# eth-cscs/conflux

Measured on AMD Instinct MI355X. Metric: fp64_lu_tflops, higher is better.
Workload: dtype f64; 1 GPU; conflux LU N=16384 v=512 grid 1x1x1 (BASELINE cfg for 1 GPU); N=16384, v=512, grid=1x1x1

## Files before the change

### conflux_amd/__init__.py

```python
import ctypes
import os

_HERE = os.path.dirname(os.path.abspath(__file__))
_LIB_PATH = os.path.join(_HERE, "libconflux_lu.so")

UID_BYTES = 128


class ConfluxLuError(RuntimeError):
    pass


def _load():
    if not os.path.exists(_LIB_PATH):
        raise ConfluxLuError(
            f"HIP engine not built: {_LIB_PATH} missing. "
            "Run `make -C conflux_amd` (or __graft_entry__.build()). "
            "The product has no CPU fallback.")
    lib = ctypes.CDLL(_LIB_PATH)
    lib.conflux_lu_create.argtypes = [ctypes.c_int] * 7 + [
        ctypes.c_char_p, ctypes.POINTER(ctypes.c_void_p)]
    lib.conflux_lu_make_uid.argtypes = [ctypes.c_char_p]
    lib.conflux_lu_init_matrix.argtypes = [ctypes.c_void_p, ctypes.c_uint64]
    lib.conflux_lu_init_matrix_spd.argtypes = [ctypes.c_void_p, ctypes.c_uint64]
# ... 7 lines not shown
    lib.conflux_lu_factor.argtypes = [ctypes.c_void_p,
                                      ctypes.POINTER(ctypes.c_double)]
    lib.conflux_lu_get_factors.argtypes = [ctypes.c_void_p, ctypes.c_void_p,
                                           ctypes.c_void_p]
    lib.conflux_lu_get_factors_sim.argtypes = [ctypes.c_void_p, ctypes.c_int,
                                               ctypes.c_void_p, ctypes.c_void_p]
    lib.conflux_lu_dims.argtypes = [ctypes.c_void_p] + [
        ctypes.POINTER(ctypes.c_int)] * 6
    lib.conflux_lu_kernel_stats.argtypes = [
        ctypes.c_void_p, ctypes.c_int, ctypes.POINTER(ctypes.c_double),
        ctypes.POINTER(ctypes.c_long), ctypes.POINTER(ctypes.c_double)]
    lib.conflux_lu_validate.argtypes = [ctypes.c_void_p,
                                        ctypes.POINTER(ctypes.c_double)]
    lib.conflux_chol_validate.argtypes = [ctypes.c_void_p,
                                          ctypes.POINTER(ctypes.c_double)]
    lib.conflux_lu_destroy.argtypes = [ctypes.c_void_p]
    lib.conflux_lu_build_info.restype = ctypes.c_char_p
    lib.conflux_lu_debug_dgemm.argtypes = [
        ctypes.c_int, ctypes.c_longlong, ctypes.c_int, ctypes.c_void_p,
        ctypes.c_void_p, ctypes.c_void_p]
    lib.conflux_lu_debug_getrf.argtypes = [ctypes.c_int, ctypes.c_int,
                                           ctypes.c_void_p, ctypes.c_void_p]
    lib.conflux_lu_debug_set_panel_glue.argtypes = [ctypes.c_int]
    lib.conflux_lu_debug_set_trsm_stripe.argtypes = [ctypes.c_int]
    lib.conflux_lu_debug_trsm_stripe_width.argtypes = []
    lib.conflux_lu_debug_trsm_ld.argtypes = [
        ctypes.c_int, ctypes.c_int, ctypes.c_int, ctypes.c_longlong,
        ctypes.c_longlong, ctypes.c_longlong, ctypes.c_void_p,
        ctypes.c_void_p]
    lib.conflux_lu_debug_dgemm_bench.argtypes = [
        ctypes.c_int, ctypes.c_longlong, ctypes.c_int, ctypes.c_int,
        ctypes.POINTER(ctypes.c_double)]
    lib.conflux_lu_debug_trsm.argtypes = [
        ctypes.c_int, ctypes.c_int, ctypes.c_longlong, ctypes.c_int,
        ctypes.c_void_p, ctypes.c_void_p]
    lib.conflux_lu_solve.argtypes = [
        ctypes.c_void_p, ctypes.c_void_p, ctypes.c_int,
        ctypes.POINTER(ctypes.c_double)]
    lib.conflux_chol_solve.argtypes = lib.conflux_lu_solve.argtypes
    lib.conflux_lu_debug_trsm_left.argtypes = [
        ctypes.c_int, ctypes.c_int, ctypes.c_int, ctypes.c_longlong,
        ctypes.c_longlong, ctypes.c_void_p, ctypes.c_void_p]
    lib.conflux_lu_debug_update_skinny.argtypes = [
        ctypes.c_int, ctypes.c_int, ctypes.c_int, ctypes.c_longlong,
        ctypes.c_void_p, ctypes.c_void_p, ctypes.c_void_p]
    lib.conflux_lu_solve_refined.argtypes = [
# ... 267 lines not shown
```

### conflux_amd/csrc/engine.cpp

```cpp
#include <hip/hip_runtime.h>
#include <rccl/rccl.h>

#include <algorithm>
#include <chrono>
#include <cmath>
#include <cstdio>
#include <cstdlib>
#include <cstring>
#include <functional>
#include <numeric>
#include <string>
#include <set>
#include <vector>

#include "../../include/conflux_lu.h"
#include "kernels.hpp"
#include "norm1est.hpp"

#define HIPCHK(x)                                                       \
    do {                                                                \
        hipError_t e_ = (x);                                            \
        if (e_ != hipSuccess) {                                         \
            std::fprintf(stderr, "[conflux_lu] HIP error %s at %s:%d\n", \
                         hipGetErrorString(e_), __FILE__, __LINE__);    \
// ... 188 lines not shown
        if (!std::isfinite(x)) {
            ++bad;
            continue;
        }
        const double a = std::fabs(x);
        if (a == 0) ++zeros;
        if (a > mx) mx = a;
        if (a < mn) mn = a;
    }
    std::fprintf(stderr,
                 "[nanscan] k=%d %-12s bad=%ld/%lld zeros=%ld min=%.3e "
                 "max=%.3e\n",
                 k, tag, bad, (long long)ns, zeros, mn, mx);
}

int g_panel_glue = -1;
int panel_glue_mode() {
    if (g_panel_glue < 0) {
        const char *e = getenv("CONFLUX_PANEL_GLUE");
        g_panel_glue = e ? (atoi(e) != 0) : 1;
    }
    return g_panel_glue;
}

int factor_panel(Ctx &c, RankState &r, int n, std::vector<int> &ipiv_out) {
    const int v = c.v;
    const int NB = conflux_panel_nb();
    const int nsteps = std::min(v, n);
    ipiv_out.assign(v, 0);
    size_t slot;
    if (ev_begin(c, 1, 0, &slot)) return CONFLUX_LU_EHIP;
    auto leaf = [&](int jb, bool perm = true) -> int {
        const int nb = std::min(NB, nsteps - jb);
        const int m = n - jb;
        if (launch_panel_factor(r.panel + i64(jb) * v + jb, v, m, nb, r.sync,
                                r.d_ipiv + jb, c.epoch, r.d_swap,
                                r.d_swap + 64, c.stream)) {
            c.err = "panel grid not resident";
            return CONFLUX_LU_EINTERNAL;
        }
        c.epoch += nb;
        if (perm && v > nb)
            launch_rowperm_skip(r.panel, v, r.d_swap, r.d_swap + 64, jb,
                                2 * nb, jb, nb, v - nb, r.rowtmp, c.stream);
        return 0;
    };
// ... 58 lines not shown
                static int glue_cap = -1;
                if (glue_cap < 0) {
                    const char *gc = getenv("CONFLUX_GLUE_CAP");
                    glue_cap = gc ? atoi(gc) : 0;
                }
                launch_dgemm_f64(r.panel + i64(jb + nb) * v + jb, v,
                                 r.panel + i64(jb) * v + jb + nb, v,
                                 r.panel + i64(jb + nb) * v + jb + nb, v,
                                 m - nb, v - jb - nb, nb, c.stream,
                                 glue_cap);
            }
        }
    }
    if (ev_end(c, slot)) return CONFLUX_LU_EHIP;
    std::vector<int> raw(v);
    unsigned int perr = 0;
    char *d_err = (char *)r.sync + conflux_panel_err_offset();
    HIPCHK(hipMemcpyAsync(raw.data(), r.d_ipiv, nsteps * 4,
                          hipMemcpyDeviceToHost, c.stream));
    HIPCHK(hipMemcpyAsync(&perr, d_err, 4, hipMemcpyDeviceToHost, c.stream));
    HIPCHK(hipStreamSynchronize(c.stream));
    if (perr) {
        HIPCHK(hipMemsetAsync(d_err, 0, 4, c.stream));
        c.err = "panel hand-off timed out: column code " +
                std::to_string(perr) + " (1 + sub-panel column)";
        return CONFLUX_LU_EINTERNAL;
    }
    for (int jb = 0; jb < nsteps; jb += NB) {
        const int nb = std::min(NB, nsteps - jb);
        for (int s = 0; s < nb; ++s) ipiv_out[jb + s] = jb + raw[jb + s];
    }
    return 0;
}

void ipiv_to_perm(const std::vector<int> &ipiv, int n, int v,
                  std::vector<int> &perm) {
    perm.resize(std::max(2 * v, n));
    std::iota(perm.begin(), perm.end(), 0);
    for (int i = 0; i < std::min(v, n); ++i) std::swap(perm[i], perm[ipiv[i]]);
}

int g_trsm_stripe = -1;
int trsm_stripe_mode() {
    if (g_trsm_stripe < 0) {
        const char *e = getenv("CONFLUX_TRSM_STRIPE");
        g_trsm_stripe = e ? (atoi(e) != 0) : 1;
    }
    return g_trsm_stripe;
}
// ... 327 lines not shown
    int rc = timed_region(c, elapsed_ms, [&]() -> int {
        StepPlan sp;
        int rc = phase01(c, 0, sp);
        if (rc) return rc;
        for (int k = 0; k < c.Nt; ++k) {
            rc = run_step(c, k, sp);
            if (rc) return rc;
        }
        return 0;
    });
    if (rc) return rc;
    static int spin_stats = -1;
    if (spin_stats < 0) {
        const char *e = getenv("CONFLUX_SPIN_STATS");
        spin_stats = e ? atoi(e) : 0;
    }
    if (spin_stats) {
        for (auto &r : c.rs) {
            unsigned long long sp2 = 0;
            conflux_panel_spin_read(r.sync, &sp2, c.stream);
            std::fprintf(stderr, "[spinstats] rank %d spins=%llu\n",
                         r.grank, sp2);
        }
    }
    if (gap_stats_on())
        std::fprintf(stderr,
                     "[gapstats] steps=%ld entry->trsm=%.3f ms  gri/igri=%.3f "
                     "ms  entry->ev_pc=%.3f ms (%ld steps)\n",
                     g_gap.steps, g_gap.to_trsm, g_gap.gri, g_gap.to_evpc,
                     g_gap.evpc_steps);
    return 0;
}

int phase01(Ctx &c, int k, StepPlan &sp) {
    const int v = c.v, Px = c.Px, Py = c.Py, Pz = c.Pz;
    const int64_t Nl = c.Nl;
    const int loff = (k / Py) * v;
    const int kcol = k % Py, krow = k % Px;
    const int n_rounds = Px > 1 ? (int)std::ceil(std::log2((double)Px)) : 0;

    for (auto &r : c.rs) {
        if (r.pj != kcol) continue;
        launch_copy2d(r.A11 + i64(r.fnp) * Nl + loff, Nl,
                      r.A10 + i64(r.fnp) * v, v, r.nact, v, c.stream);
    }
    {
// ... 2114 lines not shown
    hipEvent_t a, b;
    HIPCHK(hipEventCreate(&a));
    HIPCHK(hipEventCreate(&b));
    HIPCHK(hipEventRecord(a, s));
    for (int i = 0; i < iters; ++i)
        launch_row_gather(src, cols, dst, cols, idx, rows, cols, s);
    HIPCHK(hipEventRecord(b, s));
    HIPCHK(hipEventSynchronize(b));
    float ms = 0;
    HIPCHK(hipEventElapsedTime(&ms, a, b));
    *gbps = 2.0 * rows * (double)cols * 8 * iters / (ms * 1e-3) / 1e9;
    (void)hipFree(src); (void)hipFree(dst); (void)hipFree(idx);
    (void)hipEventDestroy(a); (void)hipEventDestroy(b);
    (void)hipStreamDestroy(s);
    return CONFLUX_LU_OK;
}

int conflux_lu_debug_set_panel_glue(int mode) {
    const int prev = panel_glue_mode();
    g_panel_glue = mode != 0;
    return prev;
}

int conflux_lu_debug_getrf(int n, int v, double *panel, int *ipiv_out) {
    Ctx c;
    c.v = v;
    HIPCHK(hipStreamCreate(&c.stream));
    RankState r;
    HIPCHK(hipMalloc(&r.panel, i64(std::max(n, 2 * v)) * v * 8));
    HIPCHK(hipMalloc(&r.d_ipiv, (v + 8) * 4));
    HIPCHK(hipMalloc(&r.d_swap, 128 * 4));
    HIPCHK(hipMalloc(&r.rowtmp, i64(64) * v * 8));
    HIPCHK(hipMalloc(&r.sync, conflux_panel_sync_bytes()));
    HIPCHK(hipMemset(r.sync, 0, conflux_panel_sync_bytes()));
    HIPCHK(hipMemcpy(r.panel, panel, i64(n) * v * 8, hipMemcpyHostToDevice));
    std::vector<int> ipiv;
    int rc = factor_panel(c, r, n, ipiv);
    if (!rc) {
        HIPCHK(hipMemcpy(panel, r.panel, i64(n) * v * 8,
                         hipMemcpyDeviceToHost));
        std::copy(ipiv.begin(), ipiv.end(), ipiv_out);
    }
    (void)hipFree(r.panel); (void)hipFree(r.d_ipiv);
    (void)hipFree(r.d_swap); (void)hipFree(r.rowtmp);
    (void)hipFree(r.sync);
    for (auto &e : c.evs) { (void)hipEventDestroy(e.a); (void)hipEventDestroy(e.b); }
// ... 285 lines not shown
```

### conflux_amd/csrc/kernels.hip

```cpp
#include <hip/hip_runtime.h>

#include <cstdint>
#include <cstdlib>

#include "kernels.hpp"

#define DEVFN __device__ __forceinline__

typedef double f64x4 __attribute__((ext_vector_type(4)));
typedef double f64x2 __attribute__((ext_vector_type(2)));
typedef double f64x2u __attribute__((ext_vector_type(2), aligned(8)));

namespace ck {

DEVFN uint64_t splitmix64(uint64_t z) {
    z += 0x9E3779B97F4A7C15ull;
    z ^= z >> 30;
    z *= 0xBF58476D1CE4E5B9ull;
    z ^= z >> 27;
    z *= 0x94D049BB133111EBull;
    z ^= z >> 31;
    return z;
}

// ... 110 lines not shown
        dst[(int64_t)(dst_idx[r] + row_base) * ldd + c] = tmp[r * tot_cols + cc];
    }
}

__global__ void k_row_move(const double *__restrict__ src, int64_t lds,
                           double *__restrict__ dst, int64_t ldd,
                           const int *__restrict__ src_idx,
                           const int *__restrict__ dst_idx, int n_rows,
                           int64_t cols) {
    const int64_t stride = (int64_t)gridDim.x * blockDim.x;
    for (int64_t i = (int64_t)blockIdx.x * blockDim.x + threadIdx.x;
         i < (int64_t)n_rows * cols; i += stride) {
        const int64_t r = i / cols, c = i % cols;
        dst[(int64_t)dst_idx[r] * ldd + c] = src[(int64_t)src_idx[r] * lds + c];
    }
}



#define PANEL_TPB 256
#define PANEL_NB 32

#define PANEL_REC (PANEL_NB + 2)
struct PanelSync2 {
    alignas(16) unsigned long long key[2][CONFLUX_PANEL_MAX_BLOCKS][2];
    alignas(16) double cand_row[2][CONFLUX_PANEL_MAX_BLOCKS][PANEL_REC];
    alignas(16) double diag_row[2][PANEL_NB];
    unsigned int err;
    unsigned long long spin_sum;
};


typedef unsigned int __attribute__((address_space(1))) gu32;
typedef unsigned long long __attribute__((address_space(1))) gu64;
#define RLX_AGENT __ATOMIC_RELAXED, __HIP_MEMORY_SCOPE_AGENT

DEVFN void st_rlx_u64(unsigned long long *p, unsigned long long v) {
    __hip_atomic_store((gu64 *)p, v, RLX_AGENT);
}
DEVFN unsigned long long ld_rlx_u64(const unsigned long long *p) {
    return __hip_atomic_load((const gu64 *)p, RLX_AGENT);
}
DEVFN void st_rlx_u32(unsigned int *p, unsigned int v) {
    __hip_atomic_store((gu32 *)p, v, RLX_AGENT);
}
DEVFN unsigned int ld_rlx_u32(const unsigned int *p) {
    return __hip_atomic_load((const gu32 *)p, RLX_AGENT);
}
DEVFN void st_rlx_f64(double *p, double v) {
    union { double d; unsigned long long u; } x;
    x.d = v;
    st_rlx_u64((unsigned long long *)p, x.u);
// ... 9 lines not shown
DEVFN void dpp_fold_first_max(double &d, int &idx) {
    union { double d; int i[2]; } s, o;
    s.d = d;
    o.i[0] = __builtin_amdgcn_update_dpp(s.i[0], s.i[0], CTRL, ROW_MASK, 0xf,
                                         false);
    o.i[1] = __builtin_amdgcn_update_dpp(s.i[1], s.i[1], CTRL, ROW_MASK, 0xf,
                                         false);
    const int oi =
        __builtin_amdgcn_update_dpp(idx, idx, CTRL, ROW_MASK, 0xf, false);
    if (o.d > d || (o.d == d && oi < idx)) {
        d = o.d;
        idx = oi;
    }
}
DEVFN void wave_first_max(double &d, int &idx) {
    dpp_fold_first_max<0x111, 0xf>(d, idx);
    dpp_fold_first_max<0x112, 0xf>(d, idx);
    dpp_fold_first_max<0x114, 0xf>(d, idx);
    dpp_fold_first_max<0x118, 0xf>(d, idx);
    dpp_fold_first_max<0x142, 0xa>(d, idx);
    dpp_fold_first_max<0x143, 0xc>(d, idx);
}

typedef int i32x4 __attribute__((ext_vector_type(4)));
union F64x2Bits {
    double d[2];
    i32x4 v;
};

__global__ __launch_bounds__(256) void k_trsm_left_lower_unit32(
    const double *__restrict__ L, int64_t ldl, double *__restrict__ X,
    int64_t ldx, int nb, int64_t N) {
    __shared__ double sL[32][33];
    const int tid = threadIdx.x;
    for (int i = tid; i < nb * nb; i += 256) sL[i / nb][i % nb] = L[(i / nb) * ldl + i % nb];
    __syncthreads();
    const int64_t j = (int64_t)blockIdx.x * 256 + tid;
    if (j >= N) return;
    double x[32];
#pragma unroll
    for (int r = 0; r < 32; ++r) x[r] = (r < nb) ? X[r * ldx + j] : 0.0;
#pragma unroll
    for (int r = 1; r < 32; ++r) {
        double acc = x[r];
#pragma unroll
        for (int i = 0; i < r; ++i) acc -= sL[r][i] * x[i];
        if (r < nb) x[r] = acc;
    }
#pragma unroll
    for (int r = 0; r < 32; ++r)
        if (r < nb) X[r * ldx + j] = x[r];
}

template <int QR, int TPB>
__global__ __launch_bounds__(TPB) void k_panel_factor(
    double *__restrict__ panel, int64_t ldp, int m, int nb,
    PanelSync2 *__restrict__ sync, int *__restrict__ ipiv,
    unsigned int epoch0, int nblocks, int *__restrict__ swap_dst,
    int *__restrict__ swap_src, int backoff) {
    constexpr int RPB = QR * TPB;
    const int tid = threadIdx.x, bid = blockIdx.x;
    const int r0 = bid * RPB + tid;
    __shared__ double rows[QR][TPB][PANEL_NB + 1];
    __shared__ double piv_lds[PANEL_NB];
    __shared__ double diag_lds[PANEL_NB];
    __shared__ double red_abs[TPB];
    __shared__ int red_row[TPB];
    __shared__ int sh_piv;
    __shared__ int sm_base[PANEL_NB];
    __shared__ int sm_opos[PANEL_NB], sm_osrc[PANEL_NB];
    __shared__ int sm_novf;
    if (bid == 0 && tid == 0) {
        for (int i = 0; i < nb; ++i) sm_base[i] = i;
        sm_novf = 0;
    }
    const auto srsrc = __builtin_amdgcn_make_buffer_rsrc(
        (void *)sync, (short)0, (int)sizeof(PanelSync2), 0x00020000);

    unsigned long long spin_acc = 0;
    const unsigned sleep_k =
        backoff == 1 ? 1u : backoff == 2 ? 2u : backoff >= 4 ? 4u : 0u;
    const unsigned spin_limit = 2000000000u / (200u + 27u * sleep_k);
    for (int q = 0; q < QR; ++q) {
        const int r = r0 + q * TPB;
        for (int cc = 0; cc < nb; ++cc)
            rows[q][tid][cc] = (r < m) ? panel[(int64_t)r * ldp + cc] : 0.0;
    }

    static_assert(PANEL_NB <= RPB,
                  "diag row pc < nb <= PANEL_NB must lie in block 0");
    auto publish_col = [&](int pc, double wa, int wrow) {
        const unsigned int pep = epoch0 + (unsigned)pc;
        const int ppar = (int)(pep & 1u);
        const int rec_off =
            (int)offsetof(PanelSync2, cand_row) +
            (ppar * CONFLUX_PANEL_MAX_BLOCKS + bid) * PANEL_REC * 8;
        if (tid == 32) {
            i32x4 rv = {wrow, 0, 0, 0};
            __builtin_amdgcn_raw_buffer_store_b128(
                rv, srsrc, rec_off + PANEL_NB * 8, 0,  16);
        }
        if (tid < 16) {
// ... 53 lines not shown
        int arow = m;
        for (int q = 0; q < QR; ++q) {
            const int r = r0 + q * TPB;
            if (r >= 0 && r < m) {
                const double a = fabs(rows[q][tid][0]);
                if (a > amax || (a == amax && r < arow)) { amax = a; arow = r; }
            }
        }
        reduce_to_partials(amax, arow);
        __syncthreads();
        double wa;
        int wrow;
        combine_partials(wa, wrow);
        publish_col(0, wa, wrow);
    }

    for (int c = 0; c < nb; ++c) {
        const unsigned int epoch = epoch0 + (unsigned)c;
        const int par = (int)(epoch & 1u);
        const int diag_off =
            (int)offsetof(PanelSync2, diag_row) + par * PANEL_NB * 8;

        if (tid < 64) {
            double a_d = -1.0;
            int a_win = 0;
            for (int b = tid; b < nblocks; b += 64) {
                unsigned long long g0, g1;
                unsigned spins = 0;
                for (;;) {
                    g0 = ld_rlx_u64(&sync->key[par][b][0]);
                    g1 = ld_rlx_u64(&sync->key[par][b][1]);
                    if ((unsigned)(g0 >> 32) == epoch &&
                        (unsigned)(g1 >> 32) == epoch)
                        break;
                    if (backoff == 1) __builtin_amdgcn_s_sleep(1);
                    else if (backoff == 2) __builtin_amdgcn_s_sleep(2);
                    else if (backoff >= 4) __builtin_amdgcn_s_sleep(4);
                    if (++spins > spin_limit) {
                        st_rlx_u32(&sync->err, 1u + (unsigned)c);
                        break;
                    }
                }
                spin_acc += spins;
                union { double d; unsigned long long u; } a;
                a.u = (g0 << 32) | (g1 & 0xffffffffull);
                if (a.d > a_d) {
                    a_d = a.d;
                    a_win = b;
                }
            }
            wave_first_max(a_d, a_win);
            const int win = __builtin_amdgcn_readlane(a_win, 63);
            __builtin_amdgcn_fence(__ATOMIC_ACQUIRE, "wavefront");
            i32x4 rec = {0, 0, 0, 0};
            if (tid == 16 || (tid < 16 && 2 * tid < nb))
                rec = __builtin_amdgcn_raw_buffer_load_b128(
                    srsrc,
                    (int)offsetof(PanelSync2, cand_row) +
                        (par * CONFLUX_PANEL_MAX_BLOCKS + win) * PANEL_REC *
                            8 +
                        16 * tid,
                    0,  16);
            if (tid < 16 && 2 * tid < nb) {
                F64x2Bits x;
                x.v = rec;
                piv_lds[2 * tid] = x.d[0];
                piv_lds[2 * tid + 1] = x.d[1];
                x.v = __builtin_amdgcn_raw_buffer_load_b128(
                    srsrc, diag_off + 16 * tid, 0,  16);
                diag_lds[2 * tid] = x.d[0];
                diag_lds[2 * tid + 1] = x.d[1];
            }
            const int w_row = __builtin_amdgcn_readlane(rec[0], 16);
            if (tid == 0) {
// ... 1 lines not shown
                if (bid == 0) {
                    ipiv[c] = w_row;
                    int *b;
                    if (w_row < nb) {
                        b = &sm_base[w_row];
                    } else {
                        int j = 0;
                        for (; j < sm_novf && sm_opos[j] != w_row; ++j) {
                        }
                        if (j == sm_novf) {
                            sm_opos[j] = w_row;
                            sm_osrc[j] = w_row;
                            ++sm_novf;
                        }
                        b = &sm_osrc[j];
                    }
                    const int t = sm_base[c];
                    sm_base[c] = *b;
                    *b = t;
                }
            }
        }
        __syncthreads();
        const int piv = sh_piv;
        const double pivval = piv_lds[c];
        const bool do_scale = pivval != 0.0;
        const double recip = do_scale ? 1.0 / pivval : 0.0;

        double namax = -1.0;
        int narow = m;
        for (int q = 0; q < QR; ++q) {
            const int r = r0 + q * TPB;
            if (r >= m) continue;
            double *my = rows[q][tid];
            if (r == c) {
                for (int cc = 0; cc < nb; ++cc) my[cc] = piv_lds[cc];
            } else if (r == piv) {
                for (int cc = 0; cc < c; ++cc) my[cc] = diag_lds[cc];
                const double v0 = diag_lds[c];
                const double l = do_scale ? v0 * recip : v0;
                my[c] = l;
                for (int cc = c + 1; cc < nb; ++cc)
                    my[cc] = diag_lds[cc] - l * piv_lds[cc];
            } else if (r > c) {
                const double l = do_scale ? my[c] * recip : my[c];
                my[c] = l;
                for (int cc = c + 1; cc < nb; ++cc)
                    my[cc] -= l * piv_lds[cc];
            }
            if (r > c && c + 1 < nb) {
                const double a = fabs(my[c + 1]);
                if (a > namax || (a == namax && r < narow)) {
                    namax = a;
                    narow = r;
                }
            }
        }
        if (c + 1 < nb) reduce_to_partials(namax, narow);
        __syncthreads();
        if (c + 1 < nb) {
            double wa;
            int wrow;
            combine_partials(wa, wrow);
            publish_col(c + 1, wa, wrow);
        }
    }

    for (int q = 0; q < QR; ++q) {
        const int r = r0 + q * TPB;
        if (r >= m) continue;
        for (int cc = 0; cc < nb; ++cc)
            panel[(int64_t)r * ldp + cc] = rows[q][tid][cc];
    }
    if (tid < 64) {
        unsigned long long t = spin_acc;
        for (int w2 = 32; w2 > 0; w2 >>= 1) t += __shfl_down(t, w2);
        if (tid == 0 && t)
            (void)__hip_atomic_fetch_add((gu64 *)&sync->spin_sum, t,
                                         RLX_AGENT);
    }
    if (bid == 0 && tid < 2 * PANEL_NB && swap_dst) {
        const int i = tid;
        int d, sv;
        if (i < nb) {
            d = i;
            sv = sm_base[i];
        } else if (i - nb < sm_novf) {
            d = sm_opos[i - nb];
            sv = sm_osrc[i - nb];
        } else {
            d = 0;
            sv = sm_base[0];
        }
        if (i < 2 * nb) {
            swap_dst[i] = d;
            swap_src[i] = sv;
        }
    }
}

__global__ __launch_bounds__(256) void k_trsm_right_upper32(
    const double *__restrict__ U, int64_t ldu, double *__restrict__ X,
    int64_t ldx, int nb, int64_t M, int trans) {
    __shared__ double sU[32][33];
    __shared__ double sX[256][33];
    const int tid = threadIdx.x;
    for (int i = tid; i < nb * nb; i += 256)
        sU[i / nb][i % nb] = trans ? U[(i % nb) * ldu + i / nb]
                                   : U[(i / nb) * ldu + i % nb];
    const int64_t r0 = (int64_t)blockIdx.x * 256;
    const int rows = (int)min((int64_t)256, M - r0);
    for (int i = tid; i < rows * nb; i += 256) sX[i / nb][i % nb] = X[(r0 + i / nb) * ldx + i % nb];
    __syncthreads();
    if (tid < rows) {
        double x[32];
#pragma unroll
        for (int c = 0; c < 32; ++c) x[c] = (c < nb) ? sX[tid][c] : 0.0;
#pragma unroll
        for (int c = 0; c < 32; ++c) {
// ... 960 lines not shown
                       dim3((unsigned)cdiv64(N, 32 * WN),                     \
                            (unsigned)cdiv64(M, 64 * WM)),                    \
                       dim3(64 * WM * WN), 0, s, A, lda, B, ldb, C, ldc, M, N)
    if (tile == 0) GLUE_UPDATE(2, 4);
    else if (tile == 1) GLUE_UPDATE(1, 4);
    else GLUE_UPDATE(2, 2);
#undef GLUE_UPDATE
}

static void panel_shape(int *qr, int *tpb) {
    static int g_qr = -1, g_tpb = 0;
    if (g_qr < 0) {
        const char *r = getenv("CONFLUX_PANEL_RPB");
        const char *t = getenv("CONFLUX_PANEL_TPB");
        g_tpb = t ? atoi(t) : 256;
        if (g_tpb != 512 && g_tpb != 128) g_tpb = 256;
        const int rpb = r ? atoi(r) : 256;
        g_qr = (rpb / g_tpb >= 2) ? 2 : 1;
    }
    *qr = g_qr;
    *tpb = g_tpb;
}

static int panel_qr() {
    int qr, tpb;
    panel_shape(&qr, &tpb);
    return qr;
}

int conflux_panel_blocks_per_cu() {
    int qr, tpb;
    panel_shape(&qr, &tpb);
    const int rows = qr * tpb;
    return rows <= 128 ? 4 : rows <= 256 ? 2 : 1;
}

int launch_panel_factor(double *panel, int64_t ldp, int m, int nb, void *sync,
                        int *ipiv, unsigned int epoch0, int *swap_dst,
                        int *swap_src, hipStream_t s) {
    static int backoff = -1;
    if (backoff < 0) {
        const char *e = getenv("CONFLUX_PANEL_SLEEP");
        backoff = e ? atoi(e) : 2;
    }
    int qr, tpb;
    panel_shape(&qr, &tpb);
    int rpb = qr * tpb;
    int nblocks = (int)cdiv64(m, rpb);
    if (nblocks < 1) nblocks = 1;
    if (nblocks > CONFLUX_PANEL_MAX_BLOCKS && rpb < 512) {
        qr = 2; tpb = 256; rpb = 512;
        nblocks = (int)cdiv64(m, rpb);
    }
    if (nblocks > CONFLUX_PANEL_MAX_BLOCKS) return -1;
    if (qr == 1 && tpb == 512)
        hipLaunchKernelGGL((k_panel_factor<1, 512>), dim3(nblocks), dim3(512),
                           0, s, panel, ldp, m, nb, (PanelSync2 *)sync, ipiv,
                           epoch0, nblocks, swap_dst, swap_src, backoff);
    else if (qr == 1 && tpb == 128)
        hipLaunchKernelGGL((k_panel_factor<1, 128>), dim3(nblocks), dim3(128),
                           0, s, panel, ldp, m, nb, (PanelSync2 *)sync, ipiv,
                           epoch0, nblocks, swap_dst, swap_src, backoff);
    else if (qr == 1)
        hipLaunchKernelGGL((k_panel_factor<1, 256>), dim3(nblocks), dim3(256),
                           0, s, panel, ldp, m, nb, (PanelSync2 *)sync, ipiv,
                           epoch0, nblocks, swap_dst, swap_src, backoff);
    else
        hipLaunchKernelGGL((k_panel_factor<2, 256>), dim3(nblocks), dim3(256),
                           0, s, panel, ldp, m, nb, (PanelSync2 *)sync, ipiv,
                           epoch0, nblocks, swap_dst, swap_src, backoff);
    return 0;
}

void conflux_panel_spin_read(void *sync, unsigned long long *out,
                             hipStream_t s) {
    (void)hipMemcpyAsync(out, (char *)sync + offsetof(PanelSync2, spin_sum),
                         8, hipMemcpyDeviceToHost, s);
    (void)hipStreamSynchronize(s);
    (void)hipMemsetAsync((char *)sync + offsetof(PanelSync2, spin_sum), 0, 8,
                         s);
}

int conflux_panel_sync_bytes() { return (int)sizeof(PanelSync2); }
int conflux_panel_err_offset() { return (int)offsetof(PanelSync2, err); }
int conflux_panel_nb() { return PANEL_NB; }
int conflux_panel_rpb() {
    int qr, tpb;
    panel_shape(&qr, &tpb);
    return qr * tpb;
}

void launch_trsm_left_lower_unit32(const double *L, int64_t ldl, double *X,
                                   int64_t ldx, int nb, int64_t N,
                                   hipStream_t s) {
    if (N <= 0 || nb <= 0) return;
    hipLaunchKernelGGL(k_trsm_left_lower_unit32, dim3(cdiv64(N, 256)),
                       dim3(256), 0, s, L, ldl, X, ldx, nb, N);
}

void launch_trsm_right_upper32(const double *U, int64_t ldu, double *X,
                               int64_t ldx, int nb, int64_t M, int trans,
                               hipStream_t s) {
    if (M <= 0 || nb <= 0) return;
    hipLaunchKernelGGL(k_trsm_right_upper32, dim3(cdiv64(M, 256)), dim3(256),
                       0, s, U, ldu, X, ldx, nb, M, trans);
// ... 691 lines not shown
```

### conflux_amd/csrc/kernels.hpp

```cpp
#pragma once
#include <hip/hip_runtime.h>

#include <cstdint>

#define CONFLUX_PANEL_MAX_BLOCKS 256

void launch_init_matrix(double *A, int Ml, int Nl, int v, int Px, int Py,
                        int pi, int pj, int zero_layer, uint64_t seed,
                        hipStream_t s);
void launch_copy2d(const double *src, int64_t lds, double *dst, int64_t ldd,
                   int rows, int64_t cols, hipStream_t s);
void launch_zero2d(double *dst, int64_t ldd, int rows, int64_t cols,
                   hipStream_t s);
void launch_add2d(const double *src, int64_t lds, double *dst, int64_t ldd,
                  int rows, int64_t cols, hipStream_t s);
void launch_row_gather(const double *src, int64_t lds, double *dst,
                       int64_t ldd, const int *idx, int n_rows, int64_t cols,
                       hipStream_t s);
void launch_row_scatter(const double *src, int64_t lds, double *dst,
                        int64_t ldd, const int *idx, int n_rows, int64_t cols,
                        hipStream_t s);
void launch_rowperm_skip(double *mat, int64_t ld, const int *dst_idx,
                         const int *src_idx, int row_base, int n_rows,
                         int64_t skip0, int64_t skipn, int64_t tot_cols,
                         double *tmp, hipStream_t s);
void launch_panel_glue_prep(double *mat, int64_t ld, const int *dst_idx,
                            const int *src_idx, int jb, int tot_cols,
                            const double *L, int64_t ldl, hipStream_t s);
void launch_panel_glue_update(const double *A, int64_t lda, const double *B,
                              int64_t ldb, double *C, int64_t ldc, int M,
                              int N, hipStream_t s);
int launch_panel_factor(double *panel, int64_t ldp, int m, int nb, void *sync,
                        int *ipiv, unsigned int epoch0, int *swap_dst,
                        int *swap_src, hipStream_t s);
int conflux_panel_sync_bytes();
int conflux_panel_err_offset();
void conflux_panel_spin_read(void *sync, unsigned long long *out,
                             hipStream_t s);
int conflux_panel_nb();
int conflux_panel_rpb();
int conflux_panel_blocks_per_cu();
void launch_trsm_left_lower_unit32(const double *L, int64_t ldl, double *X,
                                   int64_t ldx, int nb, int64_t N,
                                   hipStream_t s);
void launch_trsm_right_upper32(const double *U, int64_t ldu, double *X,
                               int64_t ldx, int nb, int64_t M, int trans,
                               hipStream_t s);
void launch_trsm_right_mfma(const double *U, int64_t ldu, double *X,
                            int64_t ldx, int v, int64_t M, int trans,
                            hipStream_t s);
void launch_trsm_left_mfma(const double *L, int64_t ldl, double *X,
                           int64_t ldx, int v, int64_t N, hipStream_t s);
int conflux_trsm_stripe_width();
bool conflux_trsm_stripe_fits(int v);
int64_t conflux_trsm_stripe_ws_doubles(int v);
void launch_trsm_right_stripe(const double *U, int64_t ldu, double *X,
                              int64_t ldx, int v, int64_t M, int trans,
                              double *ws, hipStream_t s);
void launch_trsm_left_stripe(const double *L, int64_t ldl, double *X,
                             int64_t ldx, int v, int64_t N, double *ws,
                             hipStream_t s);
// ... 62 lines not shown
```

Baseline: 18.77 TFLOP/s.

## Add register-resident panel factor kernel with optional granule-tagged publish path

Adds a new panel factorization kernel that keeps each thread's 32-column row in registers across all pivot steps, using compile-time unrolled per-column updates and DPP wave-max reductions in place of repeated LDS/global traffic. It is enabled by default when the panel shape matches (nb=32, one row per thread, 256 threads). An optional publish mode writes candidate rows as epoch-tagged 64-bit granules so readers can skip a separate store drain. Phase-timing instrumentation is also added. The register-resident row raises VGPR pressure and the switch over columns adds code size.

```diff
diff --git a/conflux_amd/__init__.py b/conflux_amd/__init__.py
--- a/conflux_amd/__init__.py
+++ b/conflux_amd/__init__.py
@@ -53,6 +53,10 @@
     lib.conflux_lu_debug_getrf.argtypes = [ctypes.c_int, ctypes.c_int,
                                            ctypes.c_void_p, ctypes.c_void_p]
     lib.conflux_lu_debug_set_panel_glue.argtypes = [ctypes.c_int]
+    lib.conflux_lu_debug_set_panel_reg.argtypes = [ctypes.c_int]
+    lib.conflux_lu_debug_set_panel_publish.argtypes = [ctypes.c_int]
+    lib.conflux_lu_debug_set_panel_phase_stats.argtypes = [ctypes.c_int]
+    lib.conflux_lu_debug_panel_phase_stats.argtypes = [ctypes.c_void_p]
     lib.conflux_lu_debug_set_trsm_stripe.argtypes = [ctypes.c_int]
     lib.conflux_lu_debug_trsm_stripe_width.argtypes = []
     lib.conflux_lu_debug_trsm_ld.argtypes = [
diff --git a/conflux_amd/csrc/engine.cpp b/conflux_amd/csrc/engine.cpp
--- a/conflux_amd/csrc/engine.cpp
+++ b/conflux_amd/csrc/engine.cpp
@@ -234,6 +234,9 @@
     }
     return g_panel_glue;
 }
+
+unsigned long long g_panel_phase_acc[8] = {0, 0, 0, 0, 0, 0, 0, 0};
+unsigned long long g_panel_phase_cols = 0;
 
 int factor_panel(Ctx &c, RankState &r, int n, std::vector<int> &ipiv_out) {
     const int v = c.v;
@@ -338,9 +341,21 @@
     HIPCHK(hipStreamSynchronize(c.stream));
     if (perr) {
         HIPCHK(hipMemsetAsync(d_err, 0, 4, c.stream));
-        c.err = "panel hand-off timed out: column code " +
-                std::to_string(perr) + " (1 + sub-panel column)";
+        if (perr >= 0x10000u)
+            c.err = "panel hand-off timed out in the granule payload "
+                    "re-read: column code " +
+                    std::to_string(perr - 0x10000u) +
+                    " (1 + sub-panel column)";
+        else
+            c.err = "panel hand-off timed out in the key poll: column code " +
+                    std::to_string(perr) + " (1 + sub-panel column)";
         return CONFLUX_LU_EINTERNAL;
+    }
+    if (conflux_panel_phase_stats_mode()) {
+        unsigned long long ph[8];
+        conflux_panel_phase_read(r.sync, ph, c.stream);
+        for (int i = 0; i < 8; ++i) g_panel_phase_acc[i] += ph[i];
+        g_panel_phase_cols += nsteps;
     }
     for (int jb = 0; jb < nsteps; jb += NB) {
         const int nb = std::min(NB, nsteps - jb);
@@ -714,6 +729,17 @@
             std::fprintf(stderr, "[spinstats] rank %d spins=%llu\n",
                          r.grank, sp2);
         }
+    }
+    if (conflux_panel_phase_stats_mode() && g_panel_phase_cols) {
+        const unsigned long long *p = g_panel_phase_acc;
+        std::fprintf(stderr,
+                     "[phasestats] cols=%llu cycles all blocks: wait=%llu "
+                     "load=%llu update=%llu publish=%llu | block 0: wait=%llu "
+                     "load=%llu update=%llu publish=%llu\n",
+                     g_panel_phase_cols, p[0], p[1], p[2], p[3], p[4], p[5],
+                     p[6], p[7]);
+        for (auto &x : g_panel_phase_acc) x = 0;
+        g_panel_phase_cols = 0;
     }
     if (gap_stats_on())
         std::fprintf(stderr,
@@ -2874,6 +2900,29 @@
     return prev;
 }
 
+int conflux_lu_debug_set_panel_reg(int mode) {
+    return conflux_panel_set_reg_mode(mode);
+}
+
+int conflux_lu_debug_set_panel_publish(int mode) {
+    return conflux_panel_set_publish_mode(mode);
+}
+
+int conflux_lu_debug_set_panel_phase_stats(int mode) {
+    return conflux_panel_set_phase_stats_mode(mode);
+}
+
+int conflux_lu_debug_panel_phase_stats(unsigned long long *out9) {
+    if (!out9) return CONFLUX_LU_EARG;
+    for (int i = 0; i < 8; ++i) {
+        out9[i] = g_panel_phase_acc[i];
+        g_panel_phase_acc[i] = 0;
+    }
+    out9[8] = g_panel_phase_cols;
+    g_panel_phase_cols = 0;
+    return CONFLUX_LU_OK;
+}
+
 int conflux_lu_debug_getrf(int n, int v, double *panel, int *ipiv_out) {
     Ctx c;
     c.v = v;
diff --git a/conflux_amd/csrc/kernels.hip b/conflux_amd/csrc/kernels.hip
--- a/conflux_amd/csrc/kernels.hip
+++ b/conflux_amd/csrc/kernels.hip
@@ -156,12 +156,18 @@
 #define PANEL_NB 32
 
 #define PANEL_REC (PANEL_NB + 2)
+#define PANEL_GR_IDX (2 * PANEL_NB)
+#define PANEL_GR_REC (2 * PANEL_NB + 2)
 struct PanelSync2 {
     alignas(16) unsigned long long key[2][CONFLUX_PANEL_MAX_BLOCKS][2];
     alignas(16) double cand_row[2][CONFLUX_PANEL_MAX_BLOCKS][PANEL_REC];
     alignas(16) double diag_row[2][PANEL_NB];
     unsigned int err;
     unsigned long long spin_sum;
+    alignas(16) unsigned long long
+        cand_gr[2][CONFLUX_PANEL_MAX_BLOCKS][PANEL_GR_REC];
+    alignas(16) unsigned long long diag_gr[2][2 * PANEL_NB];
+    unsigned long long phase[8];
 };
 
 
@@ -217,6 +223,41 @@
     dpp_fold_first_max<0x143, 0xc>(d, idx);
 }
 
+DEVFN void panel_phase_add(PanelSync2 *sync, const unsigned long long (&ph)[4],
+                           bool block0) {
+    for (int i = 0; i < 4; ++i) {
+        (void)__hip_atomic_fetch_add((gu64 *)&sync->phase[i], ph[i],
+                                     RLX_AGENT);
+        if (block0)
+            (void)__hip_atomic_fetch_add((gu64 *)&sync->phase[4 + i], ph[i],
+                                         RLX_AGENT);
+    }
+}
+
+template <int CTRL, int ROW_MASK>
+DEVFN void dpp_fold_max(double &d) {
+    union { double d; int i[2]; } s, o;
+    s.d = d;
+    o.i[0] = __builtin_amdgcn_update_dpp(s.i[0], s.i[0], CTRL, ROW_MASK, 0xf,
+                                         false);
+    o.i[1] = __builtin_amdgcn_update_dpp(s.i[1], s.i[1], CTRL, ROW_MASK, 0xf,
+                                         false);
+    d = fmax(d, o.d);
+}
+DEVFN double wave_max(double d) {
+    dpp_fold_max<0x111, 0xf>(d);
+    dpp_fold_max<0x112, 0xf>(d);
+    dpp_fold_max<0x114, 0xf>(d);
+    dpp_fold_max<0x118, 0xf>(d);
+    dpp_fold_max<0x142, 0xa>(d);
+    dpp_fold_max<0x143, 0xc>(d);
+    union { double d; int i[2]; } s, o;
+    s.d = d;
+    o.i[0] = __builtin_amdgcn_readlane(s.i[0], 63);
+    o.i[1] = __builtin_amdgcn_readlane(s.i[1], 63);
+    return o.d;
+}
+
 typedef int i32x4 __attribute__((ext_vector_type(4)));
 union F64x2Bits {
     double d[2];
@@ -247,7 +288,7 @@
         if (r < nb) X[r * ldx + j] = x[r];
 }
 
-template <int QR, int TPB>
+template <int QR, int TPB, bool STATS = false>
 __global__ __launch_bounds__(TPB) void k_panel_factor(
     double *__restrict__ panel, int64_t ldp, int m, int nb,
     PanelSync2 *__restrict__ sync, int *__restrict__ ipiv,
@@ -273,6 +314,7 @@
         (void *)sync, (short)0, (int)sizeof(PanelSync2), 0x00020000);
 
     unsigned long long spin_acc = 0;
+    unsigned long long ph[4] = {0, 0, 0, 0}, pt0 = 0, pt1 = 0, pt2 = 0;
     const unsigned sleep_k =
         backoff == 1 ? 1u : backoff == 2 ? 2u : backoff >= 4 ? 4u : 0u;
     const unsigned spin_limit = 2000000000u / (200u + 27u * sleep_k);
@@ -372,6 +414,7 @@
             (int)offsetof(PanelSync2, diag_row) + par * PANEL_NB * 8;
 
         if (tid < 64) {
+            if constexpr (STATS) pt0 = clock64();
             double a_d = -1.0;
             int a_win = 0;
             for (int b = tid; b < nblocks; b += 64) {
@@ -400,6 +443,7 @@
                 }
             }
             wave_first_max(a_d, a_win);
+            if constexpr (STATS) pt1 = clock64();
             const int win = __builtin_amdgcn_readlane(a_win, 63);
             __builtin_amdgcn_fence(__ATOMIC_ACQUIRE, "wavefront");
             i32x4 rec = {0, 0, 0, 0};
@@ -447,6 +491,8 @@
             }
         }
         __syncthreads();
+        if constexpr (STATS)
+            if (tid < 64) pt2 = clock64();
         const int piv = sh_piv;
         const double pivval = piv_lds[c];
         const bool do_scale = pivval != 0.0;
@@ -483,13 +529,25 @@
         }
         if (c + 1 < nb) reduce_to_partials(namax, narow);
         __syncthreads();
+        unsigned long long pt3 = 0;
+        if constexpr (STATS)
+            if (tid < 64) pt3 = clock64();
         if (c + 1 < nb) {
             double wa;
             int wrow;
             combine_partials(wa, wrow);
             publish_col(c + 1, wa, wrow);
         }
-    }
+        if constexpr (STATS)
+            if (tid < 64) {
+                ph[0] += pt1 - pt0;
+                ph[1] += pt2 - pt1;
+                ph[2] += pt3 - pt2;
+                ph[3] += clock64() - pt3;
+            }
+    }
+    if constexpr (STATS)
+        if (tid == 0) panel_phase_add(sync, ph, bid == 0);
 
     for (int q = 0; q < QR; ++q) {
         const int r = r0 + q * TPB;
@@ -520,6 +578,394 @@
         if (i < 2 * nb) {
             swap_dst[i] = d;
             swap_src[i] = sv;
+        }
+    }
+}
+
+#define PANEL_REG_TPB 256
+typedef double f64x2 __attribute__((ext_vector_type(2)));
+
+template <int C>
+DEVFN double panel_reg_column(double (&my)[PANEL_NB], const double *piv_lds,
+                              int r) {
+    const double pivval = piv_lds[C];
+    const bool do_scale = pivval != 0.0;
+    const double recip = do_scale ? 1.0 / pivval : 0.0;
+    if (r > C) {
+        const double l = do_scale ? my[C] * recip : my[C];
+        my[C] = l;
+#pragma unroll
+        for (int cc = C + 1; cc < PANEL_NB; ++cc)
+            my[cc] = fma(-l, piv_lds[cc], my[cc]);
+    }
+    if constexpr (C + 1 < PANEL_NB) return my[C + 1];
+    else return 0.0;
+}
+
+template <bool R2, bool STATS>
+__global__ __launch_bounds__(PANEL_REG_TPB) void k_panel_factor_reg(
+    double *__restrict__ panel, int64_t ldp, int m,
+    PanelSync2 *__restrict__ sync, int *__restrict__ ipiv,
+    unsigned int epoch0, int nblocks, int *__restrict__ swap_dst,
+    int *__restrict__ swap_src, int backoff) {
+    constexpr int TPB = PANEL_REG_TPB, NB = PANEL_NB, NW = TPB / 64;
+    const int tid = threadIdx.x, bid = blockIdx.x;
+    const int lane = tid & 63, wv = tid >> 6;
+    const int r = bid * TPB + tid;
+    const bool owns_c = bid == 0 && wv == 0;
+    __shared__ alignas(16) double piv_lds[NB];
+    __shared__ alignas(16) double diag_lds[NB];
+    __shared__ alignas(16) double stage[NW][NB];
+    __shared__ alignas(16) double stage_d[NB];
+    __shared__ double red_abs[NW];
+    __shared__ int red_row[NW];
+    __shared__ int sh_piv;
+    int sm_base_r = tid, sm_opos_r = 0, sm_osrc_r = 0, sm_novf = 0;
+    const auto srsrc = __builtin_amdgcn_make_buffer_rsrc(
+        (void *)sync, (short)0, (int)sizeof(PanelSync2), 0x00020000);
+    unsigned long long spin_acc = 0;
+    unsigned long long ph[4] = {0, 0, 0, 0}, pt0 = 0, pt1 = 0, pt2 = 0;
+    const unsigned sleep_k =
+        backoff == 1 ? 1u : backoff == 2 ? 2u : backoff >= 4 ? 4u : 0u;
+    const unsigned spin_limit = 2000000000u / (200u + 27u * sleep_k);
+    auto backoff_sleep = [&]() {
+        if (backoff == 1) __builtin_amdgcn_s_sleep(1);
+        else if (backoff == 2) __builtin_amdgcn_s_sleep(2);
+        else if (backoff >= 4) __builtin_amdgcn_s_sleep(4);
+    };
+
+    double my[NB];
+    if (r < m) {
+        const f64x2 *src = (const f64x2 *)(panel + (int64_t)r * ldp);
+#pragma unroll
+        for (int k = 0; k < NB / 2; ++k) {
+            const f64x2 t = src[k];
+            my[2 * k] = t.x;
+            my[2 * k + 1] = t.y;
+        }
+    } else {
+#pragma unroll
+        for (int cc = 0; cc < NB; ++cc) my[cc] = 0.0;
+    }
+    auto stage_row = [&](double *dst) {
+#pragma unroll
+        for (int k = 0; k < NB / 2; ++k) {
+            f64x2 t;
+            t.x = my[2 * k];
+            t.y = my[2 * k + 1];
+            ((f64x2 *)dst)[k] = t;
+        }
+    };
+    auto reduce_and_stage = [&](double amax, int dcol) {
+        const double mx = wave_max(amax);
+        const unsigned long long hit =
+            __builtin_amdgcn_ballot_w64(amax == mx);
+        const int wrow_w = mx > -1.0
+                               ? bid * TPB + wv * 64 + (int)__builtin_ctzll(hit)
+                               : m;
+        if (lane == 0) {
+            red_abs[wv] = mx;
+            red_row[wv] = wrow_w;
+        }
+        if (wrow_w < m && r == wrow_w) stage_row(stage[wv]);
+        if (owns_c && tid == dcol) stage_row(stage_d);
+    };
+    auto combine_partials = [&](double &wa, int &wrow) {
+        wa = red_abs[0];
+        wrow = red_row[0];
+        for (int w = 1; w < NW; ++w) {
+            const double oa = red_abs[w];
+            const int orr = red_row[w];
+            if (oa > wa || (oa == wa && orr < wrow)) { wa = oa; wrow = orr; }
+        }
+    };
+    auto publish_col = [&](int pc, double wa, int wrow) {
+        const unsigned int pep = epoch0 + (unsigned)pc;
+        const int ppar = (int)(pep & 1u);
+        const int wwave = wrow < m ? (wrow - bid * TPB) >> 6 : 0;
+        const unsigned long long tag = (unsigned long long)pep << 32;
+        union { double d; unsigned long long u; } a;
+        if constexpr (R2) {
+            if (tid < 32) {
+                a.d = stage[wwave][tid];
+                unsigned long long *g = &sync->cand_gr[ppar][bid][2 * tid];
+                st_rlx_u64(g, tag | (a.u >> 32));
+                st_rlx_u64(g + 1, tag | (a.u & 0xffffffffull));
+            } else if (bid == 0) {
+                a.d = stage_d[tid - 32];
+                unsigned long long *g = &sync->diag_gr[ppar][2 * (tid - 32)];
+                st_rlx_u64(g, tag | (a.u >> 32));
+                st_rlx_u64(g + 1, tag | (a.u & 0xffffffffull));
+            }
+            if (tid == 0)
+                st_rlx_u64(&sync->cand_gr[ppar][bid][PANEL_GR_IDX],
+                           tag | (unsigned long long)(unsigned)wrow);
+        } else {
+            const int rec_off =
+                (int)offsetof(PanelSync2, cand_row) +
+                (ppar * CONFLUX_PANEL_MAX_BLOCKS + bid) * PANEL_REC * 8;
+            if (tid == 32) {
+                i32x4 rv = {wrow, 0, 0, 0};
+                __builtin_amdgcn_raw_buffer_store_b128(
+                    rv, srsrc, rec_off + NB * 8, 0,  16);
+            }
+            if (tid < 16) {
+                F64x2Bits x;
+                x.d[0] = stage[wwave][2 * tid];
+                x.d[1] = stage[wwave][2 * tid + 1];
+                __builtin_amdgcn_raw_buffer_store_b128(
+                    x.v, srsrc, rec_off + 16 * tid, 0,  16);
+            } else if (tid < 32 && bid == 0) {
+                const int l = tid - 16;
+                F64x2Bits x;
+                x.d[0] = stage_d[2 * l];
+                x.d[1] = stage_d[2 * l + 1];
+                __builtin_amdgcn_raw_buffer_store_b128(
+                    x.v, srsrc,
+                    (int)offsetof(PanelSync2, diag_row) + ppar * NB * 8 +
+                        16 * l,
+                    0,  16);
+            }
+            drain_stores();
+        }
+        if (tid == 0) {
+            a.d = wa;
+            st_rlx_u64(&sync->key[ppar][bid][0], tag | (a.u >> 32));
+            st_rlx_u64(&sync->key[ppar][bid][1], tag | (a.u & 0xffffffffull));
+        }
+    };
+
+    {
+        double amax = -1.0;
+        if (r < m && fabs(my[0]) > -1.0) amax = fabs(my[0]);
+        reduce_and_stage(amax, 0);
+        __syncthreads();
+        if (tid < 64) {
+            double wa;
+            int wrow;
+            combine_partials(wa, wrow);
+            publish_col(0, wa, wrow);
+        }
+    }
+
+    for (int c = 0; c < NB; ++c) {
+        const unsigned int epoch = epoch0 + (unsigned)c;
+        const int par = (int)(epoch & 1u);
+        if (tid < 64) {
+            if constexpr (STATS) pt0 = clock64();
+            double a_d = -1.0;
+            int a_win = 0;
+            for (int b = tid; b < nblocks; b += 64) {
+                unsigned long long g0, g1;
+                unsigned spins = 0;
+                for (;;) {
+                    g0 = ld_rlx_u64(&sync->key[par][b][0]);
+                    g1 = ld_rlx_u64(&sync->key[par][b][1]);
+                    if ((unsigned)(g0 >> 32) == epoch &&
+                        (unsigned)(g1 >> 32) == epoch)
+                        break;
+                    backoff_sleep();
+                    if (++spins > spin_limit) {
+                        st_rlx_u32(&sync->err, 1u + (unsigned)c);
+                        break;
+                    }
+                }
+                spin_acc += spins;
+                union { double d; unsigned long long u; } a;
+                a.u = (g0 << 32) | (g1 & 0xffffffffull);
+                if (a.d > a_d) {
+                    a_d = a.d;
+                    a_win = b;
+                }
+            }
+            int win;
+            if (nblocks <= 64) {
+                const double mx = wave_max(a_d);
+                win = (int)__builtin_ctzll(
+                    __builtin_amdgcn_ballot_w64(a_d == mx));
+            } else {
+                wave_first_max(a_d, a_win);
+                win = __builtin_amdgcn_readlane(a_win, 63);
+            }
+            if constexpr (STATS) pt1 = clock64();
+            int w_row;
+            if constexpr (R2) {
+                const unsigned long long *src =
+                    tid < 32 ? &sync->cand_gr[par][win][2 * tid]
+                             : &sync->diag_gr[par][2 * (tid - 32)];
+                const unsigned long long *isrc =
+                    &sync->cand_gr[par][win][PANEL_GR_IDX];
+                unsigned long long g0, g1, gi;
+                unsigned spins = 0;
+                for (;;) {
+                    g0 = ld_rlx_u64(src);
+                    g1 = ld_rlx_u64(src + 1);
+                    gi = ld_rlx_u64(isrc);
+                    const bool stale = (unsigned)(g0 >> 32) != epoch ||
+                                       (unsigned)(g1 >> 32) != epoch ||
+                                       (unsigned)(gi >> 32) != epoch;
+                    if (__builtin_amdgcn_ballot_w64(stale) == 0ull) break;
+                    backoff_sleep();
+                    if (++spins > spin_limit) {
+                        if (tid == 0)
+                            st_rlx_u32(&sync->err,
+                                       0x10000u + 1u + (unsigned)c);
+                        break;
+                    }
+                }
+                spin_acc += tid == 0 ? spins : 0u;
+                union { double d; unsigned long long u; } a;
+                a.u = (g0 << 32) | (g1 & 0xffffffffull);
+                if (tid < 32) piv_lds[tid] = a.d;
+                else diag_lds[tid - 32] = a.d;
+                w_row = __builtin_amdgcn_readfirstlane((int)(unsigned)gi);
+            } else {
+                __builtin_amdgcn_fence(__ATOMIC_ACQUIRE, "wavefront");
+                i32x4 rec = {0, 0, 0, 0};
+                if (tid <= 16)
+                    rec = __builtin_amdgcn_raw_buffer_load_b128(
+                        srsrc,
+                        (int)offsetof(PanelSync2, cand_row) +
+                            (par * CONFLUX_PANEL_MAX_BLOCKS + win) *
+                                PANEL_REC * 8 +
+                            16 * tid,
+                        0,  16);
+                if (tid < 16) {
+                    F64x2Bits x;
+                    x.v = rec;
+                    piv_lds[2 * tid] = x.d[0];
+                    piv_lds[2 * tid + 1] = x.d[1];
+                    x.v = __builtin_amdgcn_raw_buffer_load_b128(
+                        srsrc,
+                        (int)offsetof(PanelSync2, diag_row) + par * NB * 8 +
+                            16 * tid,
+                        0,  16);
+                    diag_lds[2 * tid] = x.d[0];
+                    diag_lds[2 * tid + 1] = x.d[1];
+                }
+                w_row = __builtin_amdgcn_readlane(rec[0], 16);
+            }
+            if (tid == 0) {
+                sh_piv = w_row;
+                if (bid == 0) ipiv[c] = w_row;
+            }
+            if (bid == 0) {
+                int bval, j = 0;
+                if (w_row < NB) {
+                    bval = __builtin_amdgcn_readlane(sm_base_r, w_row);
+                } else {
+                    const unsigned long long hit = __builtin_amdgcn_ballot_w64(
+                        tid < sm_novf && sm_opos_r == w_row);
+                    if (hit) {
+                        j = __builtin_ctzll(hit);
+                    } else {
+                        j = sm_novf;
+                        if (tid == j) {
+                            sm_opos_r = w_row;
+                            sm_osrc_r = w_row;
+                        }
+                        ++sm_novf;
+                    }
+                    bval = __builtin_amdgcn_readlane(sm_osrc_r, j);
+                }
+                const int t = __builtin_amdgcn_readlane(sm_base_r, c);
+                if (tid == c) sm_base_r = bval;
+                if (w_row < NB) {
+                    if (tid == w_row) sm_base_r = t;
+                } else if (tid == j) {
+                    sm_osrc_r = t;
+                }
+            }
+        }
+        __syncthreads();
+        if constexpr (STATS)
+            if (tid < 64) pt2 = clock64();
+        const int piv = sh_piv;
+
+        double nxt = 0.0;
+#define PANEL_REG_CASE(C)                                                     \
+    case C:                                                                   \
+        nxt = panel_reg_column<C>(my, piv_lds, r);                            \
+        break;
+        if (r == piv && r > c) {
+#pragma unroll
+            for (int k = 0; k < NB / 2; ++k) {
+                const f64x2 t = ((const f64x2 *)diag_lds)[k];
+                my[2 * k] = t.x;
+                my[2 * k + 1] = t.y;
+            }
+        }
+        switch (c) {
+            PANEL_REG_CASE(0) PANEL_REG_CASE(1) PANEL_REG_CASE(2)
+            PANEL_REG_CASE(3) PANEL_REG_CASE(4) PANEL_REG_CASE(5)
+            PANEL_REG_CASE(6) PANEL_REG_CASE(7) PANEL_REG_CASE(8)
+            PANEL_REG_CASE(9) PANEL_REG_CASE(10) PANEL_REG_CASE(11)
+            PANEL_REG_CASE(12) PANEL_REG_CASE(13) PANEL_REG_CASE(14)
+            PANEL_REG_CASE(15) PANEL_REG_CASE(16) PANEL_REG_CASE(17)
+            PANEL_REG_CASE(18) PANEL_REG_CASE(19) PANEL_REG_CASE(20)
+            PANEL_REG_CASE(21) PANEL_REG_CASE(22) PANEL_REG_CASE(23)
+            PANEL_REG_CASE(24) PANEL_REG_CASE(25) PANEL_REG_CASE(26)
+            PANEL_REG_CASE(27) PANEL_REG_CASE(28) PANEL_REG_CASE(29)
+            PANEL_REG_CASE(30) PANEL_REG_CASE(31)
+        }
+#undef PANEL_REG_CASE
+        if (owns_c) {
+            const bool is_c = r == c;
+#pragma unroll
+            for (int cc = 0; cc < NB; ++cc)
+                my[cc] = is_c ? piv_lds[cc] : my[cc];
+        }
+        if (c + 1 < NB) {
+            double namax = -1.0;
+            if (r > c && r < m && fabs(nxt) > -1.0) namax = fabs(nxt);
+            reduce_and_stage(namax, c + 1);
+        }
+        __syncthreads();
+        unsigned long long pt3 = 0;
+        if constexpr (STATS)
+            if (tid < 64) pt3 = clock64();
+        if (c + 1 < NB && tid < 64) {
+            double wa;
+            int wrow;
+            combine_partials(wa, wrow);
+            publish_col(c + 1, wa, wrow);
+        }
+        if constexpr (STATS)
+            if (tid < 64) {
+                ph[0] += pt1 - pt0;
+                ph[1] += pt2 - pt1;
+                ph[2] += pt3 - pt2;
+                ph[3] += clock64() - pt3;
+            }
+    }
+    if constexpr (STATS)
+        if (tid == 0) panel_phase_add(sync, ph, bid == 0);
+
+    if (r < m) {
+        f64x2 *dst = (f64x2 *)(panel + (int64_t)r * ldp);
+#pragma unroll
+        for (int k = 0; k < NB / 2; ++k) {
+            f64x2 t;
+            t.x = my[2 * k];
+            t.y = my[2 * k + 1];
+            dst[k] = t;
+        }
+    }
+    if (tid < 64) {
+        unsigned long long t = spin_acc;
+        for (int w2 = 32; w2 > 0; w2 >>= 1) t += __shfl_down(t, w2);
+        if (tid == 0 && t)
+            (void)__hip_atomic_fetch_add((gu64 *)&sync->spin_sum, t,
+                                         RLX_AGENT);
+    }
+    if (bid == 0 && tid < 64 && swap_dst) {
+        const int base0 = __builtin_amdgcn_readlane(sm_base_r, 0);
+        if (tid < NB) {
+            const bool used = tid < sm_novf;
+            swap_dst[tid] = tid;
+            swap_src[tid] = sm_base_r;
+            swap_dst[NB + tid] = used ? sm_opos_r : 0;
+            swap_src[NB + tid] = used ? sm_osrc_r : base0;
         }
     }
 }
@@ -1526,6 +1972,39 @@
     *tpb = g_tpb;
 }
 
+static int g_panel_reg = -1, g_panel_publish = -1, g_panel_phase = -1;
+static int env_mode(int &g, const char *name, int dflt) {
+    if (g < 0) {
+        const char *e = getenv(name);
+        g = e ? (atoi(e) != 0) : dflt;
+    }
+    return g;
+}
+int conflux_panel_reg_mode() {
+    return env_mode(g_panel_reg, "CONFLUX_PANEL_REG", 1);
+}
+int conflux_panel_publish_mode() {
+    return env_mode(g_panel_publish, "CONFLUX_PANEL_PUBLISH", 0);
+}
+int conflux_panel_phase_stats_mode() {
+    return env_mode(g_panel_phase, "CONFLUX_PANEL_PHASE_STATS", 0);
+}
+int conflux_panel_set_reg_mode(int mode) {
+    const int prev = conflux_panel_reg_mode();
+    g_panel_reg = mode != 0;
+    return prev;
+}
+int conflux_panel_set_publish_mode(int mode) {
+    const int prev = conflux_panel_publish_mode();
+    g_panel_publish = mode != 0;
+    return prev;
+}
+int conflux_panel_set_phase_stats_mode(int mode) {
+    const int prev = conflux_panel_phase_stats_mode();
+    g_panel_phase = mode != 0;
+    return prev;
+}
+
 static int panel_qr() {
     int qr, tpb;
     panel_shape(&qr, &tpb);
@@ -1557,6 +2036,31 @@
         nblocks = (int)cdiv64(m, rpb);
     }
     if (nblocks > CONFLUX_PANEL_MAX_BLOCKS) return -1;
+    const int stats = conflux_panel_phase_stats_mode();
+    if (conflux_panel_reg_mode() && nb == PANEL_NB && m >= PANEL_NB &&
+        qr == 1 &&
+        tpb == PANEL_REG_TPB && ldp % 2 == 0 &&
+        ((uintptr_t)panel & 15u) == 0) {
+        const int r2 = conflux_panel_publish_mode();
+#define PANEL_REG_LAUNCH(R2, ST)                                              \
+    hipLaunchKernelGGL((k_panel_factor_reg<R2, ST>), dim3(nblocks),           \
+                       dim3(PANEL_REG_TPB), 0, s, panel, ldp, m,              \
+                       (PanelSync2 *)sync, ipiv, epoch0, nblocks, swap_dst,   \
+                       swap_src, backoff)
+        if (r2 && stats) PANEL_REG_LAUNCH(true, true);
+        else if (r2) PANEL_REG_LAUNCH(true, false);
+        else if (stats) PANEL_REG_LAUNCH(false, true);
+        else PANEL_REG_LAUNCH(false, false);
+#undef PANEL_REG_LAUNCH
+        return 0;
+    }
+    if (stats && qr == 1 && tpb == 256) {
+        hipLaunchKernelGGL((k_panel_factor<1, 256, true>), dim3(nblocks),
+                           dim3(256), 0, s, panel, ldp, m, nb,
+                           (PanelSync2 *)sync, ipiv, epoch0, nblocks,
+                           swap_dst, swap_src, backoff);
+        return 0;
+    }
     if (qr == 1 && tpb == 512)
         hipLaunchKernelGGL((k_panel_factor<1, 512>), dim3(nblocks), dim3(512),
                            0, s, panel, ldp, m, nb, (PanelSync2 *)sync, ipiv,
@@ -1585,6 +2089,14 @@
                          s);
 }
 
+void conflux_panel_phase_read(void *sync, unsigned long long *out8,
+                              hipStream_t s) {
+    char *p = (char *)sync + offsetof(PanelSync2, phase);
+    (void)hipMemcpyAsync(out8, p, 64, hipMemcpyDeviceToHost, s);
+    (void)hipStreamSynchronize(s);
+    (void)hipMemsetAsync(p, 0, 64, s);
+}
+
 int conflux_panel_sync_bytes() { return (int)sizeof(PanelSync2); }
 int conflux_panel_err_offset() { return (int)offsetof(PanelSync2, err); }
 int conflux_panel_nb() { return PANEL_NB; }
diff --git a/conflux_amd/csrc/kernels.hpp b/conflux_amd/csrc/kernels.hpp
--- a/conflux_amd/csrc/kernels.hpp
+++ b/conflux_amd/csrc/kernels.hpp
@@ -37,6 +37,14 @@
 int conflux_panel_err_offset();
 void conflux_panel_spin_read(void *sync, unsigned long long *out,
                              hipStream_t s);
+int conflux_panel_reg_mode();
+int conflux_panel_publish_mode();
+int conflux_panel_phase_stats_mode();
+int conflux_panel_set_reg_mode(int mode);
+int conflux_panel_set_publish_mode(int mode);
+int conflux_panel_set_phase_stats_mode(int mode);
+void conflux_panel_phase_read(void *sync, unsigned long long *out8,
+                              hipStream_t s);
 int conflux_panel_nb();
 int conflux_panel_rpb();
 int conflux_panel_blocks_per_cu();
```

Result: faster. 20.59 TFLOP/s, median of 6 (+9.7%).
